# niclasborlin/dbat

Hardware: AMD Instinct MI355X
Metric: LM iterations/sec (higher is better)
Workload: dtype f64

## Files before the change

### dbat_amd/csrc/dbat_core.hip

```cpp
#include <hip/hip_runtime.h>
#include <rocblas/rocblas.h>
#include <rocsolver/rocsolver.h>
#include <rccl/rccl.h>

#include <chrono>
#include <cmath>
#include <cstdio>
#include <cstdlib>
#include <memory>
#include <string>
#include <thread>
#include <type_traits>
#include <utility>
#include <atomic>
#include <vector>

#include "../../include/dbat_hip.h"
#include "chol_df.hpp"
#include "kernels.hpp"
#include "sig.hpp"
#include "heavy.hpp"
#include "plan.hpp"
#include "resect.hpp"
#include "robust.hpp"
// ... 156 lines not shown
        if (lds > 65536) {
            int i = 0;
            while (i < n_lds_opt_in && lds_opt_in[i].kernel != (const void *)K) ++i;
            if (i == n_lds_opt_in || lds_opt_in[i].bytes < lds) {
                if (i == 8) throw DeviceError{"internal: more kernels with over 64 KiB of LDS than the opt-in table holds"};
                HIPCHK(hipFuncSetAttribute((const void *)K, hipFuncAttributeMaxDynamicSharedMemorySize, (int)lds));
                lds_opt_in[i] = {(const void *)K, lds};
                n_lds_opt_in = std::max(n_lds_opt_in, i + 1);
            }
        }
        dbat::launch<K>(grid, block, lds, stream, std::forward<A>(args)...);
    }
    double f_lin = 0, trace_jtj = 0, lambda_lin = 0;
    int scale_lin = 0;
    bool have_lin = false;
    bool s_valid = false;
    bool s_dense_dirty = true;
    int n_res_evals = 0, n_lin = 0, n_solves = 0, n_trace_only = 0;

    ~Core() {
        for (auto &e : ev) if (e) (void)hipEventDestroy(e);
        for (auto &e : kev) if (e) (void)hipEventDestroy(e);
        for (auto &e : st_ev) if (e) (void)hipEventDestroy(e);
        dfchol.release(); dfchol_ip.release();
        if (hpin) (void)hipHostFree(hpin);
        if (nccl) (void)ncclCommDestroy(nccl);
        if (blas) rocblas_destroy_handle(blas);
        if (stream) (void)hipStreamDestroy(stream);
    }

// ... 73 lines not shown
            hv.io_dst = hv_io_dst.p; hv.io_ld = hv_io_ld.p; hv.io_pt = hv_io_pt.p; hv.pt_y = hv_pt_y.p;
            hv.grp_nb = hv_grp_nb.p; hv.grp_row = hv_grp_row.p; hv.task = hv_task.p; hv.ops = hv_ops.p;
            hv.obs0 = P.hv_obs0; hv.pt0 = P.hv_pt0; hv.ntasks = P.hv_ntasks; hv.max_batch_slots = P.hv_max_batch_slots;
        }
        if (const char *e = env_get("DBAT_HIP_GIANT_THREADS")) giant_threads = atoi(e);
        d.tile_batch = tile_batch.p; d.tile_cam_start = tile_cam_start.p; d.tile_cams = tile_cams.p;
        d.tile_io_start = tile_io_start.p; d.tile_iocols = tile_iocols.p; d.tile_cam_io = tile_cam_io.p;
        tile_io_simple.upload(P.tile_io_simple); d.tile_io_simple = P.tile_io_simple.empty() ? nullptr : tile_io_simple.p;
        use_sig = P.sg_ok && ntiles > 0 && tile_ncx <= 14;
        if (use_sig) {
            sg_chunk.upload(P.sg_chunk); sg_tile_chunk0.upload(P.sg_tile_chunk0); sg_lc.upload(P.sg_lc); sg_gcam.upload(P.sg_gcam);
            sg_nchunks = (int64_t)P.sg_chunk.size() / 8;
            sg_uv.upload(P.sg_uv);
            if (!P.uniform_w) sg_w.upload(P.sg_w);
            sig_rb = P.sg_rows_max <= 64 ? 4 : 5;
        }
        lapi("allocations and uploads of the plan");
        cams.alloc(P.nc); cams_f.alloc(P.nc);
        z.alloc(P.NZ); zt.alloc(P.NZ); dz.alloc(P.NZ); zlin.alloc(P.NZ); vtmp.alloc(P.NZ); vtmp2.alloc(P.NZ);
        xbuf.alloc(std::max<int64_t>(P.n, 1));
        ldS = ((P.NS + 1 + 7) / 8) * 8;
        d.ldS = ldS;
        const int64_t s_count = ldS * (P.NS + 1);
        red_count = s_count + 3 * P.NS + 8;
        red.alloc(red_count);
        S = red.p; g_red = S + s_count; g_c = g_red + P.NS; diagU = g_c + P.NS; red_scal = diagU + P.NS;
        ldiag.alloc(P.NS);
        {
            std::vector<int> first((size_t)P.NS, 0);
            for (int c = 0; c < P.nc; ++c)
                for (int k = 0; k < 6; ++k) first[(size_t)6 * c + k] = 6 * P.cam_first[c];
// ... 84 lines not shown
        robust_reset();
        HIPCHK(hipMemcpyAsync(z.p, P.z0.data(), P.NZ * 8, hipMemcpyHostToDevice, stream));
        HIPCHK(hipMemcpyAsync(io_fixed.p, P.io_fixed.data(), P.io_fixed.size() * 8, hipMemcpyHostToDevice, stream));
        if (d.any_prior) {
            HIPCHK(hipMemcpyAsync(z_prw.p, P.z_prw.data(), P.NZ * 8, hipMemcpyHostToDevice, stream));
            HIPCHK(hipMemcpyAsync(z_prv.p, P.z_prv.data(), P.NZ * 8, hipMemcpyHostToDevice, stream));
        }
        HIPCHK(hipStreamSynchronize(stream));
        if (uv_pre && io_changed && nobs > 0) {
            HIPCHK(hipMemcpy(cm_uv.p, P.cm_uv.data(), P.cm_uv.size() * 8, hipMemcpyHostToDevice));
            if (use_sig && sg_nchunks > 0) HIPCHK(hipMemcpy(sg_uv.p, P.sg_uv.data(), P.sg_uv.size() * 8, hipMemcpyHostToDevice));
            d.o_uv = o_uv.p;
            precompute_image_side();
            HIPCHK(hipStreamSynchronize(stream));
        }
        cams_at_lin = false; have_lin = false; s_valid = false; pend_build = false; lin_pending = false;
        lambda_lin = 0; scale_lin = 0; f_lin = 0; trace_jtj = 0; near_singular = false; chol_in_place = false; replicate_next = false;
        n_res_evals = n_lin = n_solves = n_trace_only = 0;
    }

    static int env_grid_obs() { return std::min(std::max(1, env_int("DBAT_HIP_GRID_OBS", 1536)), 1 << 20); }

    int64_t tile_kernel_mfma() const {
        if (route == TileRoute::none) return 0;
        int64_t n = 0;
        if (route == TileRoute::sig) {
            for (int64_t t = 0; t < ntiles; ++t) {
                const int nio = tile_ncx > 6 ? P.tile_io_start[t + 1] - P.tile_io_start[t] : 0;
                for (int64_t q = P.sg_tile_chunk0[t]; q < P.sg_tile_chunk0[t + 1]; ++q) {
                    const int npts = P.sg_chunk[8 * q + 1], k = P.sg_chunk[8 * q + 2];
                    const int ppr = std::min(SIG_PPR, 64 / std::max(k, 1)), rbk = (6 * k + nio + 1 + 15) >> 4;
// ... 95 lines not shown
    void read_scal(double *host, int n) {
        if (n <= 32) {
            HIPCHK(hipMemcpyAsync(hpin, scal.p, n * sizeof(double), hipMemcpyDeviceToHost, stream));
            sync();
            memcpy(host, hpin, n * sizeof(double));
            return;
        }
        HIPCHK(hipMemcpyAsync(host, scal.p, n * sizeof(double), hipMemcpyDeviceToHost, stream));
        sync();
    }
    void prep_cams(const double *zz, CamRec *into = nullptr) {
        if (!into) { into = cams.p; cams_at_lin = false; }
        launch<k_cam_prep>(dim3((unsigned)cdiv(P.nc, 64)), dim3(64), 0, d, zz, into);
    }
    void x_to_z(const double *x_host, double *z_dev) {
        HIPCHK(hipMemcpyAsync(z_dev, P.z0.data(), P.NZ * 8, hipMemcpyHostToDevice, stream));
        if (P.n) {
            HIPCHK(hipMemcpyAsync(xbuf.p, x_host, P.n * 8, hipMemcpyHostToDevice, stream));
            launch<k_scatter_x>(dim3((unsigned)cdiv(P.n, 256)), dim3(256), 0, P.n, x2z.p, xbuf.p, z_dev);
        }
    }
    void z_to_x(const double *z_dev, double *x_host) {
        if (!P.n) return;
        stage(4);
        z_dev = gathered(z_dev);
        launch<k_gather_x>(dim3((unsigned)cdiv(P.n, 256)), dim3(256), 0, P.n, x2z.p, z_dev, xbuf.p);
        HIPCHK(hipMemcpyAsync(x_host, xbuf.p, P.n * 8, hipMemcpyDeviceToHost, stream));
        sync();
    }

// ... 25 lines not shown
        if (!P.n || nt <= 0) return std::max(nt, 0);
        HIPCHK(hipMemcpyAsync(host, trace_dev.p, (size_t)P.n * nt * 8, hipMemcpyDeviceToHost, stream));
        HIPCHK(hipStreamSynchronize(stream));
        for (int k = 0; k < nt; ++k)
            if (!trace_have[k]) std::fill(host + (size_t)P.n * k, host + (size_t)P.n * (k + 1), NAN);
        if ((size_t)P.n * trace_cap * 8 > ((size_t)256 << 20)) {
            DevBuf<double> old;
            std::swap(old.p, trace_dev.p);
            trace_cap = 0;
        }
        return nt;
    }

    double eval_f_step(const double *x, double alpha, const double *pdir, double *out) {
        stage(3);
        if ((int64_t)cdiv(P.NZ, 256) < P.nc) { axpby(1.0, x, alpha, pdir, out); return eval_f(out, nullptr, nullptr); }
        launch<k_axpby_cams>(dim3((unsigned)cdiv(P.NZ, 256)), dim3(256), 0, d, 1.0, x, alpha, pdir, out, cams_f.p);
        return eval_f(out, nullptr, nullptr, true);
    }
    double eval_f(const double *zz, double *r_w_out, double *r_unw_out, bool cams_ready = false) {
        stage(3);
        if (!cams_ready) prep_cams(zz, cams_f.p);
        mark(6);
        const bool res_tail = n_cm_chunks_all > 0 && n_cm_chunks_all <= 512 && !d.any_prior && !multi() && !r_w_out && !r_unw_out;
        with_value<2, 3, 4, 5>(P.model, [&](auto M) {
            with_value<false, true>(uv_pre, [&](auto PRE) {
                if (n_cm_chunks_all > 0)
                    launch<k_residual_cm<M, PRE>>(dim3((unsigned)n_cm_chunks_all), dim3(256), 0, d, zz, cams_f.p, cm_pt.p, cm_uv.p, pw ? cm_w.p : (const double *)nullptr,
                                                  cm_chunk_cam.p, cm_chunk_start.p, partial.p, res_tail ? gctr.p + 1 : (unsigned *)nullptr, scal.p, hpin, res_tail ? ++mb_seq : 0ull);
                mark(7);
// ... 52 lines not shown
        else launch<k_det_round_cam<15>>(dim3((unsigned)P.nc + 1), dim3(256), 0, d, cams.p, nio, S, g_red);
    }

    void cam_normal(const double *zz, int64_t q0, int64_t nq, int ncx) {
        const double *w = pw ? cm_w.p : (const double *)nullptr;
        with_value<2, 3, 4, 5>(P.model, [&](auto M) { with_value<6, 14, 15>(ncx, [&](auto NCX) {
            if constexpr (NCX == 6)
                launch<k_cam_normal6<M>>(dim3((unsigned)nq), dim3(256), 0, d, zz, cams.p, cm_pt.p, cm_uv.p, w, cm_chunk_cam.p + q0, cm_chunk_start.p + q0, S, g_c, g_red, diagU);
            else
                launch<k_cam_normal<M, NCX>>(dim3((unsigned)nq), dim3(256), 0, d, zz, cams.p, cm_pt.p, cm_uv.p, w, cm_chunk_cam.p + q0, cm_chunk_start.p + q0, S, g_c, g_red, diagU);
        }); });
    }

    void build_enqueue(const double *zz, double lambda, int scale) {
        stage(0);
        const bool fused_first = !s_dense_dirty && P.NS >= P.nc;
        if (!fused_first) prep_cams(zz);
        else cams_at_lin = false;
        bool pivmm_set = false;
        if (s_dense_dirty) {
            HIPCHK(hipMemsetAsync(red.p, 0, red_count * sizeof(double), stream));
            s_dense_dirty = false;
        } else {
            launch<k_envelope_cams>(dim3((unsigned)P.NS), dim3(256), 0, d, zz, cams.p, S, ldS, (int)P.NS, env_tail0, col_bend.p, g_red, pivmm.p);
            pivmm_set = true;
        }
        if (!pivmm_set) HIPCHK(hipMemcpyAsync(pivmm.p, hpin + 48, 4 * sizeof(double), hipMemcpyHostToDevice, stream));
        int64_t npart = 0;
        const bool det_list = deterministic && route != TileRoute::sig;
        const int64_t nb_tiled = det_list ? 0 : P.nb_tiled;
// ... 124 lines not shown
        do_allreduce(g_c, 2 * P.NS + 8);
    }
    void trace_only_pass(const double *zz) {
        stage(0);
        prep_cams(zz);
        if (n_cm_chunks_all > 0) {
            with_value<2, 3, 4, 5>(P.model, [&](auto M) { with_value<6, 14, 15, MAXCOL>(tile_ncx, [&](auto NCX) {
                launch<k_trace_cm<M, NCX>>(dim3((unsigned)n_cm_chunks_all), dim3(256), 0, d, zz, cams.p, cm_pt.p, cm_uv.p, pw ? cm_w.p : (const double *)nullptr,
                                           cm_chunk_cam.p, cm_chunk_start.p, partial.p);
            }); });
        }
        launch<k_trace_tail>(dim3(grid_zs), dim3(1024), 0, d, gpart.p, gctr.p + 6, (const double *)partial.p, n_cm_chunks_all, hpin, ++mb_seq);
        mb_armed = true; lin_pending = true;
        sync();
        pend_build = false;
        lambda_lin = NAN; have_lin = false; s_valid = false;
        ++n_trace_only;
    }
    void build(const double *zz, double lambda, int scale, bool lazy = false, bool trace_only = false) {
        if (trace_only && !multi() && P.nranks == 1) { trace_only_pass(zz); return; }
        pend_build = false;
        trace_only = trace_only && use_sig && ntiles > 0;
        d.trace_only = trace_only ? 1 : 0;
        try { build_enqueue(zz, lambda, scale); } catch (...) { d.trace_only = 0; throw; }
        d.trace_only = 0;
        if (mg_subtree) allreduce_vectors();
        else allreduce_system();
        finish_enqueue(zz, lambda, scale);
        if (mg_subtree && replicate_next && multi()) allreduce_matrix();
        cams_at_lin = true;
        lin_pending = true;
// ... 17 lines not shown
        launch<k_finish>(dim3((unsigned)cdiv(P.NS, 256)), dim3(256), 0, d, zz, lambda, scale, S, g_c, g_red, diagU, jn2c.p, dscale.p,
                gpart.p, gctr.p + 3, (const double *)red_scal, scal.p, hpin, mg_subtree && multi() ? (const uint8_t *)z_mine.p : (const uint8_t *)nullptr,
                ride ? info.p : (int *)nullptr, ride ? df_ctl : (int *)nullptr, ride ? df_q : (unsigned long long *)nullptr, ride ? df_nq : 0);
        if (ride) dfchol.reset_done = true;
        if (scale)
            launch<k_envelope_op>(dim3((unsigned)P.NS), dim3(256), 0, S, ldS, (int)P.NS, env_tail0, col_bend.p, (const double *)dscale.p, (double *)nullptr,
                                  (unsigned long long *)nullptr);
    }

    int factor_solve_enqueue() {
        if (mg_subtree && !multi())
            throw UsageError{"this handle is one of several shards: attach a communicator (dbat_hip_comm_init) or an all-reduce "
                             "callback (dbat_hip_set_allreduce) before linearising or solving"};
        stage(1);
        mark(2);
        if (use_perm && !chol_in_place && mg_subtree && multi()) {
            dfchol.solve_domain(stream, S, ldS, linv.p, info.p, ldiag.p);
            mark(8);
            do_allreduce(dfchol.top_tiles(), dfchol.top_tiles_count());
            mark(9);
            dfchol.solve_top(stream, ldS, rhs.p, linv.p, info.p, ldiag.p, dscale.p, dz.p);
        } else if (use_perm && !chol_in_place) dfchol.solve(stream, S, ldS, rhs.p, linv.p, info.p, ldiag.p, dscale.p, dz.p);
        else dfchol_ip.solve(stream, S, ldS, rhs.p, linv.p, info.p, ldiag.p, dscale.p, dz.p);
        HIPCHK(hipGetLastError());
        if (env_df_trace) (use_perm && !chol_in_place ? dfchol : dfchol_ip).dump_trace(stream, env_df_trace);
        mark(3);
        ++n_solves;
        return 0;
    }
    void backsub_enqueue() {
        stage(2);
        mark(4);
        const bool sig_bs = use_sig && P.sg_backsub_ok;
        const int64_t b_first = sig_bs ? P.nb_tiled : 0;
        const int64_t n_sig_wg = sig_bs ? cdiv(sg_nchunks, 4) : 0;
        if (n_sig_wg > 0) {
            with_value<2, 3, 4, 5>(P.model, [&](auto M) { with_value<6, 14>(tile_ncx, [&](auto NCX) {
                launch<k_backsub_sig<M, NCX>>(dim3((unsigned)n_sig_wg), dim3(256), 0, d, zlin.p, cams.p, Vinv.p, gp.p, dz.p, partial.p + 2 * (nb + ngiant), sg_chunk.p,
                                              (int)sg_nchunks, sg_gcam.p, sg_uv.p, pw ? sg_w.p : (const double *)nullptr);
            }); });
        }
        if (nb > b_first) {
            with_value<2, 3, 4, 5>(P.model, [&](auto M) { with_value<6, 14, 15, MAXCOL>(tile_ncx, [&](auto NCX) {
                launch<k_backsub<M, NCX>>(dim3((unsigned)(nb - b_first)), dim3(P.BT), lds_back, d, zlin.p, cams.p, Vinv.p, gp.p, dz.p, partial.p, (int)b_first);
            }); });
        }
        if (ngiant > 0) {
            with_value<2, 3, 4, 5>(P.model, [&](auto M) { with_value<false, true>(P.with_io, [&](auto IO) {
                launch<k_backsub_giant<M, IO>>(dim3((unsigned)ngiant), dim3(giant_threads), 0, d, zlin.p, cams.p, Vinv.p, gp.p, dz.p, partial.p + 2 * nb);
            }); });
        }
        mark(5);
        launch<k_prior_jv>(dim3(grid_zs), dim3(1024), 0, d, zlin.p, dz.p, g_c, gp.p, gpart.p, gctr.p + 4,
                (const double *)(partial.p + 2 * b_first), nb - b_first + ngiant + n_sig_wg, (const double *)ldiag.p, pivmm.p,
                (const int *)info.p, scal.p, multi() ? (double *)nullptr : hpin, ++mb_seq,
                mg_subtree && multi() ? (const uint8_t *)piv_have.p : (const uint8_t *)nullptr);
    }
    bool near_singular = false;
    const bool pivot_stats = env_on("DBAT_HIP_PIVOT_STATS");
    double rcond_est = 0.0;
    int chol_info = 0;
    double piv_last[4] = {0, 0, 0, 0};
    bool solve(double &JpJp, double &rJp, double &pp) {
        ensure_build();
        if (!s_valid) build(zlin.p, lambda_lin, scale_lin);
        s_valid = false;
        factor_solve_enqueue();
        if (!cams_at_lin) { prep_cams(zlin.p); cams_at_lin = true; }
        backsub_enqueue();
        int hinfo = 0;
        unsigned long long hmm[4];
        const int nsl = multi() ? 4 * P.nranks : 0;
        std::vector<double> h((size_t)8 + nsl);
        if (nsl) {
            HIPCHK(hipMemcpyAsync(hpin + 40, pivmm.p, sizeof(hmm), hipMemcpyDeviceToHost, stream));
            HIPCHK(hipMemcpyAsync(hpin + 44, info.p, sizeof(hinfo), hipMemcpyDeviceToHost, stream));
            HIPCHK(hipMemsetAsync(scal.p + 8, 0, (size_t)nsl * sizeof(double), stream));
            HIPCHK(hipMemcpyAsync(scal.p + 8 + 4 * P.rank, pivmm.p, 4 * sizeof(double), hipMemcpyDeviceToDevice, stream));
            do_allreduce(scal.p, 8 + nsl);
            read_scal(h.data(), 8 + nsl);
        } else {
            mb_armed = true;
            sync();
            memcpy(h.data(), hpin, 8 * sizeof(double));
        }
        memcpy(hmm, hpin + 40, sizeof(hmm));
        memcpy(&hinfo, hpin + 44, sizeof(hinfo));
        JpJp = h[0] + h[4]; rJp = h[1] + h[5]; pp = h[6];
        double mm[4];
        memcpy(mm, hmm, sizeof(mm));
        double pmin = std::min(mm[0], mm[2]), pmax = std::max(mm[1], mm[3]);
        for (int r = 0; r < nsl / 2; ++r) { pmin = std::min(pmin, h[8 + 2 * r]); pmax = std::max(pmax, h[8 + 2 * r + 1]); }
        const bool failed = hinfo != 0 || (nsl && h[7] > 0) || !std::isfinite(pp) || !std::isfinite(JpJp);
        if (failed && !(use_perm && !chol_in_place)) s_dense_dirty = true;
        const double ratio = pmax > 0 ? pmin / pmax : 0.0;
        near_singular = failed || !(ratio * ratio >= 2.220446049250313e-16);
        rcond_est = failed ? 0.0 : ratio * ratio;
        chol_info = hinfo;
        for (int q = 0; q < 4; ++q) piv_last[q] = mm[q];
// ... 363 lines not shown
    void robust_omega_ip(double *host) {
        if (!robust_on) { std::fill(host, host + P.no, 1.0); return; }
        DevBuf<double> t;
        t.alloc((size_t)std::max<int64_t>(P.no, 1));
        HIPCHK(hipMemsetAsync(t.p, 0, (size_t)P.no * sizeof(double), stream));
        if (nobs > 0) launch<k_scatter_rows1>(dim3(robust_grid()), dim3(256), 0, nobs, (const int64_t *)o_row.p, (const double *)omega.p, t.p);
        if (multi()) do_allreduce(t.p, P.no);
        HIPCHK(hipMemcpyAsync(host, t.p, (size_t)P.no * sizeof(double), hipMemcpyDeviceToHost, stream));
        HIPCHK(hipStreamSynchronize(stream));
    }
    void jtimes(const double *v, double &JvJv, double &rJv, double &vv) {
        if (!cams_at_lin) { prep_cams(zlin.p); cams_at_lin = true; }
        with_value<2, 3, 4, 5>(P.model, [&](auto M) { with_value<6, 14, 15, MAXCOL>(tile_ncx, [&](auto NCX) {
            launch<k_jtimes<M, NCX>>(dim3(grid_obs), dim3(256), 0, d, zlin.p, cams.p, v, partial.p);
        }); });
        launch<k_prior_jv>(dim3(grid_zs), dim3(1024), 0, d, zlin.p, v, g_c, gp.p, gpart.p, gctr.p + 4,
                (const double *)partial.p, (int64_t)grid_obs, (const double *)nullptr, pivmm.p, (const int *)info.p, scal.p, (double *)nullptr, 0ull, (const uint8_t *)nullptr);
        do_allreduce(scal.p, 8);
        double h[8];
        read_scal(h, 8);
        JvJv = h[0] + h[4]; rJv = h[1] + h[5]; vv = h[6];
    }
    double dot_owned(const double *a, const double *b) {
        launch<k_dot>(dim3(grid_z), dim3(256), 0, P.NZ, z_mine.p, a, b, partial.p);
        launch<k_sum_partials<1>>(dim3(1), dim3(1024), 0, partial.p, (int64_t)grid_z, scal.p, 0);
        do_allreduce(scal.p, 1);
        double s;
        read_scal(&s, 1);
        return s;
    }
    void axpby(double a, const double *x, double b, const double *y2, double *y) {
        launch<k_axpby>(dim3((unsigned)cdiv(P.NZ, 256)), dim3(256), 0, P.NZ, a, x, b, y2, y);
    }
    void gradient(double *g) {
        launch<k_gradient>(dim3((unsigned)cdiv(P.NZ, 256)), dim3(256), 0, d, g_c, gp.p, g);
    }
    void colnorm2(double *out) {
        launch<k_jn2>(dim3((unsigned)cdiv(P.NZ, 256)), dim3(256), 0, d, jn2c.p, jn2p.p, out);
    }
    void jac_blocks(const double *zz, double *a, double *b, double *cc) {
        with_value<2, 3, 4, 5>(P.model, [&](auto M) { launch<k_jac_blocks<M>>(dim3((unsigned)cdiv(nobs, 256)), dim3(256), 0, d, zz, cams.p, a, b, cc); });
    }
    void copy(double *dst, const double *src) { HIPCHK(hipMemcpyAsync(dst, src, P.NZ * 8, hipMemcpyDeviceToDevice, stream)); }
    void accept_trial() { std::swap(z.p, zt.p); }
};


struct LoopOut {
    std::vector<double> res, damp, aux;
    int code = 0, iters = 0;
    double f_final = 0;
};

static void export_residuals(Core &c, const double *zdev, double *r_unw, double *r_wgt, double *f);
static void jtimes_rows(Core &c, const double *v_dev, double *Jv);

static void keep_Jp(Core &c, const dbat_hip_options &o, const double *p_dev, std::vector<double> &Jp) {
    if (!o.term_fun) return;
    Jp.resize((size_t)c.P.m);
// ... 95 lines not shown
    double f = c.eval_f(c.z.p, nullptr, nullptr);
    c.build(c.z.p, 0.0, 0, false, lambda0_needs_trace(o));
    const double nx = (double)c.P.n;
    double lambda0 = o.lambda0, lambdaMin = o.lambda_min;
    if (lambda0 < 0) lambda0 = std::fabs(lambda0) * c.trace_jtj / nx;
    if (lambdaMin < 0) lambdaMin = std::fabs(lambdaMin) * c.trace_jtj / nx;
    double lambda = lambda0;
    if (lambda < lambdaMin) lambda = 0;
    out.damp.push_back(lambda);
    double prevLambda = NAN;
    double JpJp = 0, rJp = 0, pp = 0;
    std::vector<double> Jp_host;
    while (true) {
        while (n <= o.max_iter) {
            if (c.lambda_lin != lambda) c.build(c.z.p, lambda, 0, true);
            const bool failed = c.solve(JpJp, rJp, pp);
            if (!failed) keep_Jp(c, o, c.dz.p, Jp_host);
            out.res.push_back(std::sqrt(2 * f));
            if (n == 0 && !c.P.rank_ok) { out.code = -4; break; }
            if (failed) { out.code = -2; break; }
            out.damp.push_back(lambda);
            trace_line(o, n, out.res.back(), n == 0 ? NAN : lambda);
            if (o.store_trace) c.trace_put(n, c.z.p);
            ++n;
            const double fNew = c.eval_f_step(c.z.p, 1.0, c.dz.p, c.zt.p);
            if (fNew < f && !vetoed(c, o)) {
                c.accept_trial();
                lambda = lambda / 10;
                if (lambda < lambdaMin) lambda = 0;
                c.request_build(lambda, 0);
                f = fNew;
// ... 17 lines not shown
static void loop_lmp(Core &c, const dbat_hip_options &o, double delta0, LoopOut &out) {
    int n = 0;
    double delta = delta0;
    std::vector<double> rhos, steps;
    if (o.store_trace) c.trace_put(0, c.z.p);
    double f = c.eval_f(c.z.p, nullptr, nullptr);
    c.build(c.z.p, 0.0, 1);
    bool have_gn = false;
    std::vector<double> Jp_host;
    double gnJpJp = 0, gnrJp = 0, gnpp = 0;
    double *pGN = c.vtmp.p, *g = c.vtmp2.p;
    while (true) {
        out.res.push_back(std::sqrt(2 * f));
        if (n == 0 && !c.P.rank_ok) { out.code = -4; break; }
        if (!have_gn) {
            const bool failed = c.solve(gnJpJp, gnrJp, gnpp);
            if (failed) { out.code = -2; break; }
            c.copy(pGN, c.dz.p);
            have_gn = true;
        }
        int step;
        double JpJp, rJp;
        const double npGN = std::sqrt(gnpp);
        if (npGN <= delta) {
            step = 0; c.copy(c.dz.p, pGN); JpJp = gnJpJp; rJp = gnrJp;
        } else {
            c.gradient(g);
            double gJJg, rJg, gg;
            c.jtimes(g, gJJg, rJg, gg);
            const double lambdaStar = gg / gJJg;
            const double nCP = lambdaStar * std::sqrt(gg);
            if (nCP > delta) {
                step = 2;
                c.axpby(-delta / std::sqrt(gg), g, 0.0, g, c.dz.p);
            } else {
                step = 1;
                const double cp_pgn = -lambdaStar * c.dot_owned(g, pGN);
                const double cp2 = nCP * nCP;
                const double A = cp2 - 2 * cp_pgn + gnpp;
                const double B = 2 * (cp_pgn - cp2);
// ... 831 lines not shown
}

int dbat_hip_bench_step(dbat_hip_handle *h, double lambda, int32_t scale_columns, double *ms) {
    API_TRY
    if (!h) { g_err = "null handle"; return DBAT_HIP_EINVAL; }
    Core &c = *h->core;
    DeviceGuard dev_guard(c.device);
    c.timing = true;
    HIPCHK(hipEventRecord(c.ev[0], c.stream));
    c.build_enqueue(c.z.p, lambda, scale_columns);
    if (c.mg_subtree) c.allreduce_vectors(); else c.allreduce_system();
    c.finish_enqueue(c.z.p, lambda, scale_columns);
    HIPCHK(hipEventRecord(c.ev[1], c.stream));
    c.factor_solve_enqueue();
    HIPCHK(hipEventRecord(c.ev[2], c.stream));
    c.backsub_enqueue();
    c.do_allreduce(c.scal.p, 8);
    HIPCHK(hipEventRecord(c.ev[3], c.stream));
    (void)c.eval_f_step(c.z.p, 1.0, c.dz.p, c.zt.p);
    HIPCHK(hipEventRecord(c.ev[4], c.stream));
    c.sync();
    c.timing = false;
    c.have_lin = true; c.lambda_lin = lambda; c.scale_lin = scale_columns; c.s_valid = false;
    if (ms) {
        for (int i = 0; i < 4; ++i) {
            float t = 0;
            HIPCHK(hipEventElapsedTime(&t, c.ev[i], c.ev[i + 1]));
            ms[i] = t;
        }
        for (int i = 0; i < 4; ++i) {
            float t = 0;
// ... 391 lines not shown
```

### dbat_amd/csrc/env.hpp

```cpp
#pragma once
#include <cstdlib>
#include <cstring>
#include <string>

extern char **environ;

namespace dbat {

#ifdef DBAT_HIP_PROFILING
constexpr bool kProfilingBuild = true;
#else
constexpr bool kProfilingBuild = false;
#endif

struct EnvSwitch { const char *name; bool measurement; const char *what; const char *values = nullptr; };
static const EnvSwitch kEnvSwitches[] = {
    {"DBAT_HIP_SIG", false, "0: signature kernels off, 2: on wherever a chunk's rows fit (default: by group length)", "0|1|2"},
    {"DBAT_HIP_SIG_IOS_OFF", false, "self-calibration: IO rows by LDS atomics in every tile"},
    {"DBAT_HIP_CMAX", false, "cameras per tile (0: column-list kernel only)"},
    {"DBAT_HIP_BT", false, "observations per batch (128 | 256)", "128|256"},
    {"DBAT_HIP_TILE_BMIN", false, "fewest batches a tile may be capped at (default 2)"},
    {"DBAT_HIP_HEAVY", false, "0: heavy / giant points by the column-list kernels (pair terms by global atomics) instead of the matrix-core path", "0|1"},
    {"DBAT_HIP_HEAVY_KS", false, "heavy / giant points: k-steps per task of k_heavy_syrk at most (default: by the amount of work, 12 ... 96)"},
    {"DBAT_HIP_GIANT_THREADS", false, "threads of the giant-point kernels (64 | 128 | 256)", "64|128|256"},
    {"DBAT_HIP_MG_REPLICATED", false, "several ranks: envelope summed, replicated factorisation"},
    {"DBAT_HIP_ND_OFF", false, "no nested dissection"},
    {"DBAT_HIP_ND_LEAF", false, "leaf size of the dissection"},
    {"DBAT_HIP_ND_PAD_ALL", false, "every block of the dissection on a tile boundary"},
    {"DBAT_HIP_ND_JOIN_SMALL", false, "separators up to that many rows join their child's last tile"},
    {"DBAT_HIP_DF_SPLIT", false, "factorisation: helper tasks for sums longer than this many products (default 96)"},
    {"DBAT_HIP_DF_CHUNK", false, "factorisation: products per helper task (default 32)"},
    {"DBAT_HIP_DF_CHAIN", false, "factorisation: 0 = diagonal tiles as ordinary tasks (no chain role), 1 = chain role whatever the pattern", "0|1"},
// ... 50 lines not shown
```

### dbat_amd/csrc/kernels.hpp

```cpp
#pragma once
#include <hip/hip_runtime.h>

#include "model.hpp"

namespace dbat {

struct DevProblem {
    int nc, np, nIOrows, nK, nP, nIOu, ncolmax, BT;
    int64_t NS, NZ, nobs, nb;
    int64_t ldS;
    const int32_t *cam_ncol, *cam_col, *cam_iorow;
    const uint32_t *cam_eo_est;
    const int32_t *io_src;
    const double *io_fixed;
    const double *px;
    const double *cam_w;
    const uint8_t *z_est, *z_mine;
    const double *z_prw, *z_prv;
    const int32_t *o_cam, *o_pt;
    const double *o_uv;
    const double *o_uv_raw;
    int uv_pre;
    const double *o_w;
    const uint32_t *o_seg;
// ... 2678 lines not shown
    const int cam = d.o_cam[o], pt = d.o_pt[o];
    const CamRec &C = cams[cam];
    const int ncol = WITH_IO ? min(C.ncol, NCX) : 6;
    double r[2], E[2][NCX], B[2][3];
    eval_obs_cols_n<MODEL, NCX>(d, C, z, o, pt, r, E, B);
    const double *vp = v + d.NS + 3 * (int64_t)pt;
    double j0 = B[0][0] * vp[0] + B[0][1] * vp[1] + B[0][2] * vp[2];
    double j1 = B[1][0] * vp[0] + B[1][1] * vp[1] + B[1][2] * vp[2];
#pragma unroll
    for (int a = 0; a < NCX; ++a)
        if (a < ncol) { const double vc = v[C.col[a]]; j0 += E[0][a] * vc; j1 += E[1][a] * vc; }
    const int64_t row = d.o_row[o];
    Jv[2 * row] = j0; Jv[2 * row + 1] = j1;
}

__global__ __launch_bounds__(1024) void k_prior_jv(DevProblem d, const double *__restrict__ z,
                                                  const double *__restrict__ v, const double *__restrict__ g_c,
                                                  const double *__restrict__ gp, double *__restrict__ partial,
                                                  unsigned *__restrict__ ctr, const double *__restrict__ bs_partial,
                                                  int64_t nbs, const double *__restrict__ ldiag,
                                                  unsigned long long *__restrict__ pivmm, const int *__restrict__ info,
                                                  double *__restrict__ out, double *__restrict__ mailbox,
                                                  unsigned long long seq, const uint8_t *__restrict__ piv_have = nullptr) {
    __shared__ double sh[80];
    double acc[5] = {0, 0, 0, 0, 0};
    const int64_t stride = (int64_t)gridDim.x * blockDim.x;
    double pmin = 1e300, pmax = 0.0;
    for (int64_t i = (int64_t)blockIdx.x * blockDim.x + threadIdx.x; i < d.NZ; i += stride) {
        if (ldiag && i < d.NS && d.z_est[i] && (!piv_have || piv_have[i])) {
            double p = ldiag[i];
            p = p == p ? p : 0.0;
            pmin = fmin(pmin, p); pmax = fmax(pmax, p);
        }
        if (!d.z_mine[i]) continue;
        const double w = d.any_prior ? d.z_prw[i] : 0.0, vi = d.z_est[i] ? v[i] : 0.0;
        if (w > 0) acc[0] += w * vi * vi;
        acc[1] += (i < d.NS ? g_c[i] : gp[i - d.NS]) * vi;
        acc[2] += vi * vi;
    }
    if (ldiag && (int64_t)blockIdx.x * blockDim.x < d.NS) {
        for (int off = 32; off > 0; off >>= 1) {
            pmin = fmin(pmin, __shfl_down(pmin, off, 64));
            pmax = fmax(pmax, __shfl_down(pmax, off, 64));
        }
        if ((threadIdx.x & 63) == 0 && pmax > 0.0) {
            atomicMin(pivmm + 2, (unsigned long long)__double_as_longlong(fmax(pmin, 0.0)));
            atomicMax(pivmm + 3, (unsigned long long)__double_as_longlong(pmax));
        }
        __builtin_amdgcn_s_waitcnt(0);
    }
    if (grid_sum<5, 2, 3>(acc, sh, partial, ctr, bs_partial, nbs, 2) && threadIdx.x == 0) {
        out[0] = acc[3]; out[1] = acc[4]; out[4] = acc[0]; out[5] = acc[1]; out[6] = acc[2];
        out[7] = info && __hip_atomic_load(info, __ATOMIC_RELAXED, __HIP_MEMORY_SCOPE_AGENT) != 0 ? 1.0 : 0.0;
        out[2] = 0.0; out[3] = 0.0;
        if (mailbox) {
            mailbox[0] = acc[3]; mailbox[1] = acc[4]; mailbox[4] = acc[0]; mailbox[5] = acc[1]; mailbox[6] = acc[2];
            for (int q = 0; q < 4; ++q)
                mailbox[40 + q] = __longlong_as_double((long long)__hip_atomic_load(pivmm + q, __ATOMIC_RELAXED, __HIP_MEMORY_SCOPE_AGENT));
            const int hi = __hip_atomic_load(info, __ATOMIC_RELAXED, __HIP_MEMORY_SCOPE_AGENT);
            long long w = hi;
            mailbox[44] = __longlong_as_double(w);
            mailbox_done(mailbox, seq);
        }
    }
}

__global__ __launch_bounds__(256) void k_dot(int64_t n, const uint8_t *__restrict__ mine,
                                             const double *__restrict__ a, const double *__restrict__ b ,
                                             double *__restrict__ partial) {
    __shared__ double sh[8];
// ... 4 lines not shown
    block_sum<1>(acc, sh);
    if (threadIdx.x == 0) partial[blockIdx.x] = acc[0];
}

__global__ void k_axpby(int64_t n, double a, const double *__restrict__ x, double b,
                        const double *__restrict__ y2, double *__restrict__ y) {
    const int64_t i = (int64_t)blockIdx.x * blockDim.x + threadIdx.x;
    if (i < n) y[i] = a * x[i] + b * y2[i];
}
__global__ void k_axpby_cams(DevProblem d, double a, const double *__restrict__ x, double b,
                             const double *__restrict__ y2, double *__restrict__ y, CamRec *__restrict__ cams) {
    const int64_t i = (int64_t)blockIdx.x * blockDim.x + threadIdx.x;
    if (i < d.NZ) y[i] = a * x[i] + b * y2[i];
    if (threadIdx.x == blockDim.x - 1 && (int)blockIdx.x < d.nc)
        cam_prep_one(d, [=](int64_t q) { return a * x[q] + b * y2[q]; }, (int)blockIdx.x, cams);
}

__global__ void k_gradient(DevProblem d, const double *__restrict__ g_c, const double *__restrict__ gp,
                           double *__restrict__ g) {
    const int64_t i = (int64_t)blockIdx.x * blockDim.x + threadIdx.x;
    if (i >= d.NZ) return;
    double v = 0;
    if (d.z_est[i]) v = i < d.NS ? g_c[i] : (d.z_mine[i] ? gp[i - d.NS] : 0.0);
    g[i] = v;
}

__global__ void k_jn2(DevProblem d, const double *__restrict__ jn2c, const double *__restrict__ jn2p,
                      double *__restrict__ out) {
    const int64_t i = (int64_t)blockIdx.x * blockDim.x + threadIdx.x;
    if (i >= d.NZ) return;
// ... 64 lines not shown
```

### dbat_amd/csrc/sig.hpp

```cpp
#pragma once
#include <cstddef>
#include <type_traits>

#include "kernels.hpp"

namespace dbat {

constexpr int SIG_LDK = 18;
constexpr int SIG_PPR = 6;
constexpr int SIG_KMAXR = 13;
constexpr int SIG_NW = 8;
constexpr int SIG_CAMW = (int)(offsetof(CamRec, ncol) / 8) + 1;
constexpr int SIG_CAMW_IO = (int)((sizeof(CamRec) + 7) / 8);
constexpr int SIG_STILE = 8064;
#ifndef DBAT_SIG_IO_WAVES
#define DBAT_SIG_IO_WAVES 4
#endif
constexpr int SIG_IO_CAMS = DBAT_SIG_IO_WAVES == 8 ? 16 : 21;
__host__ __device__ constexpr int sig_stile(bool io) { return io && DBAT_SIG_IO_WAVES == 8 ? 6336 : SIG_STILE; }
__host__ __device__ constexpr int sig_cams(bool io) { return io ? SIG_IO_CAMS : 21; }

struct SigLds {
    int next_chunk, abort_;
    int flush_turn;
// ... 655 lines not shown
        int ios = 0;
        if constexpr (NCX > 6) ios = d.tile_io_simple ? d.tile_io_simple[tile] : 0;
#ifdef DBAT_SIG_ONLY_IOS
        ios = DBAT_SIG_ONLY_IOS;
#endif
        if (NCX > 6 && ios == 1)
            build_sig_tile<MODEL, RB, NCX, (NCX > 6 ? 1 : 0), PW>(d, tile, (int)ti, z, cams, lambda, scale, S, g_red, Vinv, gp, jn2p, partial, pivmm, sg_chunk, sg_tile_chunk0, sg_lc, sg_uv, sg_w, tile_ctr + 2, sy, sh);
        else if (NCX > 6 && ios == 2)
            build_sig_tile<MODEL, RB, NCX, (NCX > 6 ? 2 : 0), PW>(d, tile, (int)ti, z, cams, lambda, scale, S, g_red, Vinv, gp, jn2p, partial, pivmm, sg_chunk, sg_tile_chunk0, sg_lc, sg_uv, sg_w, tile_ctr + 2, sy, sh);
        else
            build_sig_tile<MODEL, RB, NCX, 0, PW>(d, tile, (int)ti, z, cams, lambda, scale, S, g_red, Vinv, gp, jn2p, partial, pivmm, sg_chunk, sg_tile_chunk0, sg_lc, sg_uv, sg_w, tile_ctr + 2, sy, sh);
        __syncthreads();
    }
}

template <int MODEL, int NCX>
__global__ __launch_bounds__(256) void k_backsub_sig(DevProblem d, const double *__restrict__ z,
                                                     const CamRec *__restrict__ cams,
                                                     const double *__restrict__ Vinv, const double *__restrict__ gp,
                                                     double *__restrict__ dz, double *__restrict__ partial ,
                                                     const int32_t *__restrict__ sg_chunk, int nchunks,
                                                     const int32_t *__restrict__ sg_gcam,
                                                     const double *__restrict__ sg_uv, const double *__restrict__ sg_w) {
    constexpr int CW = (int)((sizeof(CamRec) + 7) / 8);
    __shared__ double sh[8];
    __shared__ double crec[4][SIG_KMAXR][CW];
    __shared__ double dcs[4][SIG_KMAXR][NCX];
    const int t = threadIdx.x, lane = t & 63;
    const int wv = t >> 6;
    const int ch = __builtin_amdgcn_readfirstlane(blockIdx.x * 4 + (t >> 6));
    double acc[2] = {0, 0};
    if (ch < nchunks) {
        const int32_t *cd = sg_chunk + 8 * (int64_t)ch;
        const int pt0 = cd[0], npts = cd[1], k = cd[2], gm = cd[4], gi0 = cd[5], uv0 = cd[6];
        const int mycam = lane < k ? sg_gcam[16 * (int64_t)ch + lane] : 0;
        for (int base = 0; base < k * CW; base += 64) {
            const int idx = base + lane, c = min(idx / CW, k - 1), f = idx - c * CW;
            const int cam = __builtin_amdgcn_ds_bpermute(4 * c, mycam);
            if (idx < k * CW) crec[wv][c][f] = reinterpret_cast<const double *>(cams + cam)[f];
        }
        __builtin_amdgcn_wave_barrier();
        for (int idx = lane; idx < k * NCX; idx += 64) {
            const int c = idx / NCX, a = idx - c * NCX;
            const CamRec &C = *reinterpret_cast<const CamRec *>(crec[wv][c]);
            const bool on = a < (NCX > 6 ? min(C.ncol, NCX) : 6) && (NCX > 6 || ((C.eo_est >> a) & 1u));
            dcs[wv][c][a] = on ? dz[C.col[a]] : 0.0;
// ... 44 lines not shown
#pragma unroll
            for (int c = 0; c < 6; ++c) V0[c] += lane_get(V0[c], lane ^ m);
            tt2 += lane_get(tt2, lane ^ m);
        }
        {
            const double s0 = gp[3 * (int64_t)pt] + sB[0], s1 = gp[3 * (int64_t)pt + 1] + sB[1], s2 = gp[3 * (int64_t)pt + 2] + sB[2];
            double p0, p1, p2;
            point_block_solve_neg(Vinv + 6 * (int64_t)pt, s0, s1, s2, p0, p1, p2);
            const double d0 = (est & 1u) ? p0 : 0.0, d1 = (est & 2u) ? p1 : 0.0, d2 = (est & 4u) ? p2 : 0.0;
            if (act && lane == pi) {
                dz[zp] = d0; dz[zp + 1] = d1; dz[zp + 2] = d2;
                acc[0] = tt2 + 2.0 * (d0 * sB[0] + d1 * sB[1] + d2 * sB[2])
                       + d0 * (V0[0] * d0 + V0[1] * d1 + V0[2] * d2) + d1 * (V0[1] * d0 + V0[3] * d1 + V0[4] * d2)
                       + d2 * (V0[2] * d0 + V0[4] * d1 + V0[5] * d2);
            }
        }
    }
    block_sum<2>(acc, sh);
    if (t == 0) { partial[2 * blockIdx.x] = acc[0]; partial[2 * blockIdx.x + 1] = acc[1]; }
}

}
```

Measured before the change: 634.4.

## Fuse trial-step objective evaluation into signature back-substitution kernel

When the solve is followed by a full-step objective evaluation, the back-substitution kernel now also forms the trial point coordinates, re-evaluates the residuals at the trial cameras and points, and accumulates the trial objective, with the prior term added in the prior/Jv reduction kernel. A small kernel prepares trial camera records before the back-substitution. The later eval_f_step call then reads the cached value from the mailbox instead of launching separate residual kernels, saving a pass over the observations and a host round trip. Validity flags are reset on every path that modifies z, dz, zt or the linearisation, which adds state-tracking complexity and puts extra work and register pressure on the back-substitution kernel.

```diff
diff --git a/dbat_amd/csrc/dbat_core.hip b/dbat_amd/csrc/dbat_core.hip
--- a/dbat_amd/csrc/dbat_core.hip
+++ b/dbat_amd/csrc/dbat_core.hip
@@ -194,6 +194,10 @@
     double f_lin = 0, trace_jtj = 0, lambda_lin = 0;
     int scale_lin = 0;
     bool have_lin = false;
+    bool trial_ok = false, trial_read = false;
+    double trial_f = 0;
+    bool fused_trial = true;
+    bool sg_all_points = false;
     bool s_valid = false;
     bool s_dense_dirty = true;
     int n_res_evals = 0, n_lin = 0, n_solves = 0, n_trace_only = 0;
@@ -297,7 +301,11 @@
             sg_uv.upload(P.sg_uv);
             if (!P.uniform_w) sg_w.upload(P.sg_w);
             sig_rb = P.sg_rows_max <= 64 ? 4 : 5;
-        }
+            int64_t npts = 0;
+            for (int64_t q = 0; q < sg_nchunks; ++q) npts += P.sg_chunk[8 * q + 1];
+            sg_all_points = npts == (int64_t)P.np;
+        }
+        fused_trial = env_int("DBAT_HIP_FUSED_TRIAL", 1) != 0;
         lapi("allocations and uploads of the plan");
         cams.alloc(P.nc); cams_f.alloc(P.nc);
         z.alloc(P.NZ); zt.alloc(P.NZ); dz.alloc(P.NZ); zlin.alloc(P.NZ); vtmp.alloc(P.NZ); vtmp2.alloc(P.NZ);
@@ -412,7 +420,7 @@
             precompute_image_side();
             HIPCHK(hipStreamSynchronize(stream));
         }
-        cams_at_lin = false; have_lin = false; s_valid = false; pend_build = false; lin_pending = false;
+        cams_at_lin = false; have_lin = false; trial_ok = false; s_valid = false; pend_build = false; lin_pending = false;
         lambda_lin = 0; scale_lin = 0; f_lin = 0; trace_jtj = 0; near_singular = false; chol_in_place = false; replicate_next = false;
         n_res_evals = n_lin = n_solves = n_trace_only = 0;
     }
@@ -538,6 +546,7 @@
         launch<k_cam_prep>(dim3((unsigned)cdiv(P.nc, 64)), dim3(64), 0, d, zz, into);
     }
     void x_to_z(const double *x_host, double *z_dev) {
+        trial_ok = false;
         HIPCHK(hipMemcpyAsync(z_dev, P.z0.data(), P.NZ * 8, hipMemcpyHostToDevice, stream));
         if (P.n) {
             HIPCHK(hipMemcpyAsync(xbuf.p, x_host, P.n * 8, hipMemcpyHostToDevice, stream));
@@ -593,6 +602,13 @@
 
     double eval_f_step(const double *x, double alpha, const double *pdir, double *out) {
         stage(3);
+        if (trial_ok && alpha == 1.0 && x == z.p && pdir == dz.p && out == zt.p) {
+            mark(6); mark(7);
+            if (!trial_read) { mb_armed = true; sync(); trial_f = hpin[8]; trial_read = true; }
+            ++n_res_evals;
+            return 0.5 * trial_f;
+        }
+        trial_ok = false;
         if ((int64_t)cdiv(P.NZ, 256) < P.nc) { axpby(1.0, x, alpha, pdir, out); return eval_f(out, nullptr, nullptr); }
         launch<k_axpby_cams>(dim3((unsigned)cdiv(P.NZ, 256)), dim3(256), 0, d, 1.0, x, alpha, pdir, out, cams_f.p);
         return eval_f(out, nullptr, nullptr, true);
@@ -675,6 +691,7 @@
 
     void build_enqueue(const double *zz, double lambda, int scale) {
         stage(0);
+        trial_ok = false;
         const bool fused_first = !s_dense_dirty && P.NS >= P.nc;
         if (!fused_first) prep_cams(zz);
         else cams_at_lin = false;
@@ -829,7 +846,7 @@
         mb_armed = true; lin_pending = true;
         sync();
         pend_build = false;
-        lambda_lin = NAN; have_lin = false; s_valid = false;
+        lambda_lin = NAN; have_lin = false; trial_ok = false; s_valid = false;
         ++n_trace_only;
     }
     void build(const double *zz, double lambda, int scale, bool lazy = false, bool trace_only = false) {
@@ -877,6 +894,7 @@
                              "callback (dbat_hip_set_allreduce) before linearising or solving"};
         stage(1);
         mark(2);
+        trial_ok = false;
         if (use_perm && !chol_in_place && mg_subtree && multi()) {
             dfchol.solve_domain(stream, S, ldS, linv.p, info.p, ldiag.p);
             mark(8);
@@ -891,16 +909,26 @@
         ++n_solves;
         return 0;
     }
-    void backsub_enqueue() {
+    bool trial_fusable() const {
+        return fused_trial && use_sig && P.sg_backsub_ok && sg_nchunks > 0 && sg_all_points && nb == P.nb_tiled && ngiant == 0 &&
+               (tile_ncx == 6) == uv_pre && !deterministic && !multi() && P.nranks == 1;
+    }
+    void backsub_enqueue(bool want_trial = false) {
         stage(2);
         mark(4);
+        const bool fuse = want_trial && trial_fusable();
+        trial_ok = false;
+        if (fuse) launch<k_trial_cams>(dim3((unsigned)cdiv(P.NS, 256)), dim3(256), 0, d, zlin.p, dz.p, zt.p, cams_f.p);
         const bool sig_bs = use_sig && P.sg_backsub_ok;
         const int64_t b_first = sig_bs ? P.nb_tiled : 0;
         const int64_t n_sig_wg = sig_bs ? cdiv(sg_nchunks, 4) : 0;
         if (n_sig_wg > 0) {
             with_value<2, 3, 4, 5>(P.model, [&](auto M) { with_value<6, 14>(tile_ncx, [&](auto NCX) {
-                launch<k_backsub_sig<M, NCX>>(dim3((unsigned)n_sig_wg), dim3(256), 0, d, zlin.p, cams.p, Vinv.p, gp.p, dz.p, partial.p + 2 * (nb + ngiant), sg_chunk.p,
-                                              (int)sg_nchunks, sg_gcam.p, sg_uv.p, pw ? sg_w.p : (const double *)nullptr);
+                with_value<false, true>(fuse, [&](auto TR) {
+                    launch<k_backsub_sig<M, NCX, TR>>(dim3((unsigned)n_sig_wg), dim3(256), 0, d, zlin.p, cams.p, Vinv.p, gp.p, dz.p, partial.p + 2 * (nb + ngiant), sg_chunk.p,
+                                                      (int)sg_nchunks, sg_gcam.p, sg_uv.p, pw ? sg_w.p : (const double *)nullptr,
+                                                      TR ? zt.p : (double *)nullptr, TR ? cams_f.p : (const CamRec *)nullptr);
+                });
             }); });
         }
         if (nb > b_first) {
@@ -914,23 +942,26 @@
             }); });
         }
         mark(5);
-        launch<k_prior_jv>(dim3(grid_zs), dim3(1024), 0, d, zlin.p, dz.p, g_c, gp.p, gpart.p, gctr.p + 4,
-                (const double *)(partial.p + 2 * b_first), nb - b_first + ngiant + n_sig_wg, (const double *)ldiag.p, pivmm.p,
-                (const int *)info.p, scal.p, multi() ? (double *)nullptr : hpin, ++mb_seq,
-                mg_subtree && multi() ? (const uint8_t *)piv_have.p : (const uint8_t *)nullptr);
+        with_value<false, true>(fuse, [&](auto TR) {
+            launch<k_prior_jv<TR>>(dim3(grid_zs), dim3(1024), 0, d, zlin.p, dz.p, g_c, gp.p, gpart.p, gctr.p + 4,
+                    (const double *)(partial.p + 2 * b_first), nb - b_first + ngiant + n_sig_wg, (const double *)ldiag.p, pivmm.p,
+                    (const int *)info.p, scal.p, multi() ? (double *)nullptr : hpin, ++mb_seq,
+                    mg_subtree && multi() ? (const uint8_t *)piv_have.p : (const uint8_t *)nullptr);
+        });
+        trial_ok = fuse; trial_read = false;
     }
     bool near_singular = false;
     const bool pivot_stats = env_on("DBAT_HIP_PIVOT_STATS");
     double rcond_est = 0.0;
     int chol_info = 0;
     double piv_last[4] = {0, 0, 0, 0};
-    bool solve(double &JpJp, double &rJp, double &pp) {
+    bool solve(double &JpJp, double &rJp, double &pp, bool want_trial = false) {
         ensure_build();
         if (!s_valid) build(zlin.p, lambda_lin, scale_lin);
         s_valid = false;
         factor_solve_enqueue();
         if (!cams_at_lin) { prep_cams(zlin.p); cams_at_lin = true; }
-        backsub_enqueue();
+        backsub_enqueue(want_trial);
         int hinfo = 0;
         unsigned long long hmm[4];
         const int nsl = multi() ? 4 * P.nranks : 0;
@@ -946,6 +977,7 @@
             mb_armed = true;
             sync();
             memcpy(h.data(), hpin, 8 * sizeof(double));
+            if (trial_ok) { trial_f = hpin[8]; trial_read = true; }
         }
         memcpy(hmm, hpin + 40, sizeof(hmm));
         memcpy(&hinfo, hpin + 44, sizeof(hinfo));
@@ -1339,7 +1371,7 @@
         with_value<2, 3, 4, 5>(P.model, [&](auto M) { with_value<6, 14, 15, MAXCOL>(tile_ncx, [&](auto NCX) {
             launch<k_jtimes<M, NCX>>(dim3(grid_obs), dim3(256), 0, d, zlin.p, cams.p, v, partial.p);
         }); });
-        launch<k_prior_jv>(dim3(grid_zs), dim3(1024), 0, d, zlin.p, v, g_c, gp.p, gpart.p, gctr.p + 4,
+        launch<k_prior_jv<false>>(dim3(grid_zs), dim3(1024), 0, d, zlin.p, v, g_c, gp.p, gpart.p, gctr.p + 4,
                 (const double *)partial.p, (int64_t)grid_obs, (const double *)nullptr, pivmm.p, (const int *)info.p, scal.p, (double *)nullptr, 0ull, (const uint8_t *)nullptr);
         do_allreduce(scal.p, 8);
         double h[8];
@@ -1355,6 +1387,7 @@
         return s;
     }
     void axpby(double a, const double *x, double b, const double *y2, double *y) {
+        trial_ok = false;
         launch<k_axpby>(dim3((unsigned)cdiv(P.NZ, 256)), dim3(256), 0, P.NZ, a, x, b, y2, y);
     }
     void gradient(double *g) {
@@ -1366,8 +1399,11 @@
     void jac_blocks(const double *zz, double *a, double *b, double *cc) {
         with_value<2, 3, 4, 5>(P.model, [&](auto M) { launch<k_jac_blocks<M>>(dim3((unsigned)cdiv(nobs, 256)), dim3(256), 0, d, zz, cams.p, a, b, cc); });
     }
-    void copy(double *dst, const double *src) { HIPCHK(hipMemcpyAsync(dst, src, P.NZ * 8, hipMemcpyDeviceToDevice, stream)); }
-    void accept_trial() { std::swap(z.p, zt.p); }
+    void copy(double *dst, const double *src) {
+        if (dst == z.p || dst == zt.p || dst == dz.p || dst == zlin.p) trial_ok = false;
+        HIPCHK(hipMemcpyAsync(dst, src, P.NZ * 8, hipMemcpyDeviceToDevice, stream));
+    }
+    void accept_trial() { std::swap(z.p, zt.p); trial_ok = false; }
 };
 
 
@@ -1493,7 +1529,7 @@
     while (true) {
         while (n <= o.max_iter) {
             if (c.lambda_lin != lambda) c.build(c.z.p, lambda, 0, true);
-            const bool failed = c.solve(JpJp, rJp, pp);
+            const bool failed = c.solve(JpJp, rJp, pp, true);
             if (!failed) keep_Jp(c, o, c.dz.p, Jp_host);
             out.res.push_back(std::sqrt(2 * f));
             if (n == 0 && !c.P.rank_ok) { out.code = -4; break; }
@@ -1541,7 +1577,7 @@
         out.res.push_back(std::sqrt(2 * f));
         if (n == 0 && !c.P.rank_ok) { out.code = -4; break; }
         if (!have_gn) {
-            const bool failed = c.solve(gnJpJp, gnrJp, gnpp);
+            const bool failed = c.solve(gnJpJp, gnrJp, gnpp, true);
             if (failed) { out.code = -2; break; }
             c.copy(pGN, c.dz.p);
             have_gn = true;
@@ -1550,7 +1586,8 @@
         double JpJp, rJp;
         const double npGN = std::sqrt(gnpp);
         if (npGN <= delta) {
-            step = 0; c.copy(c.dz.p, pGN); JpJp = gnJpJp; rJp = gnrJp;
+            step = 0; JpJp = gnJpJp; rJp = gnrJp;
+            if (!c.trial_ok) c.copy(c.dz.p, pGN);
         } else {
             c.gradient(g);
             double gJJg, rJg, gg;
@@ -2412,7 +2449,7 @@
     HIPCHK(hipEventRecord(c.ev[1], c.stream));
     c.factor_solve_enqueue();
     HIPCHK(hipEventRecord(c.ev[2], c.stream));
-    c.backsub_enqueue();
+    c.backsub_enqueue(true);
     c.do_allreduce(c.scal.p, 8);
     HIPCHK(hipEventRecord(c.ev[3], c.stream));
     (void)c.eval_f_step(c.z.p, 1.0, c.dz.p, c.zt.p);
diff --git a/dbat_amd/csrc/env.hpp b/dbat_amd/csrc/env.hpp
--- a/dbat_amd/csrc/env.hpp
+++ b/dbat_amd/csrc/env.hpp
@@ -16,6 +16,7 @@
 struct EnvSwitch { const char *name; bool measurement; const char *what; const char *values = nullptr; };
 static const EnvSwitch kEnvSwitches[] = {
     {"DBAT_HIP_SIG", false, "0: signature kernels off, 2: on wherever a chunk's rows fit (default: by group length)", "0|1|2"},
+    {"DBAT_HIP_FUSED_TRIAL", false, "0: the objective at the full step by its own kernels behind the solve, not inside the back-substitution", "0|1"},
     {"DBAT_HIP_SIG_IOS_OFF", false, "self-calibration: IO rows by LDS atomics in every tile"},
     {"DBAT_HIP_CMAX", false, "cameras per tile (0: column-list kernel only)"},
     {"DBAT_HIP_BT", false, "observations per batch (128 | 256)", "128|256"},
diff --git a/dbat_amd/csrc/kernels.hpp b/dbat_amd/csrc/kernels.hpp
--- a/dbat_amd/csrc/kernels.hpp
+++ b/dbat_amd/csrc/kernels.hpp
@@ -2716,6 +2716,7 @@
     Jv[2 * row] = j0; Jv[2 * row + 1] = j1;
 }
 
+template <bool TRIAL>
 __global__ __launch_bounds__(1024) void k_prior_jv(DevProblem d, const double *__restrict__ z,
                                                   const double *__restrict__ v, const double *__restrict__ g_c,
                                                   const double *__restrict__ gp, double *__restrict__ partial,
@@ -2724,8 +2725,9 @@
                                                   unsigned long long *__restrict__ pivmm, const int *__restrict__ info,
                                                   double *__restrict__ out, double *__restrict__ mailbox,
                                                   unsigned long long seq, const uint8_t *__restrict__ piv_have = nullptr) {
-    __shared__ double sh[80];
-    double acc[5] = {0, 0, 0, 0, 0};
+    constexpr int NV = TRIAL ? 6 : 5;
+    __shared__ double sh[16 * NV];
+    double acc[NV] = {};
     const int64_t stride = (int64_t)gridDim.x * blockDim.x;
     double pmin = 1e300, pmax = 0.0;
     for (int64_t i = (int64_t)blockIdx.x * blockDim.x + threadIdx.x; i < d.NZ; i += stride) {
@@ -2739,6 +2741,8 @@
         if (w > 0) acc[0] += w * vi * vi;
         acc[1] += (i < d.NS ? g_c[i] : gp[i - d.NS]) * vi;
         acc[2] += vi * vi;
+        if constexpr (TRIAL)
+            if (w > 0) { const double e = (z[i] + v[i]) - d.z_prv[i]; acc[5] += w * e * e; }
     }
     if (ldiag && (int64_t)blockIdx.x * blockDim.x < d.NS) {
         for (int off = 32; off > 0; off >>= 1) {
@@ -2751,11 +2755,12 @@
         }
         __builtin_amdgcn_s_waitcnt(0);
     }
-    if (grid_sum<5, 2, 3>(acc, sh, partial, ctr, bs_partial, nbs, 2) && threadIdx.x == 0) {
+    if (grid_sum<NV, NV - 3, 3>(acc, sh, partial, ctr, bs_partial, nbs, NV - 3) && threadIdx.x == 0) {
         out[0] = acc[3]; out[1] = acc[4]; out[4] = acc[0]; out[5] = acc[1]; out[6] = acc[2];
         out[7] = info && __hip_atomic_load(info, __ATOMIC_RELAXED, __HIP_MEMORY_SCOPE_AGENT) != 0 ? 1.0 : 0.0;
-        out[2] = 0.0; out[3] = 0.0;
+        out[2] = TRIAL ? acc[NV - 1] : 0.0; out[3] = 0.0;
         if (mailbox) {
+            if constexpr (TRIAL) mailbox[8] = acc[NV - 1];
             mailbox[0] = acc[3]; mailbox[1] = acc[4]; mailbox[4] = acc[0]; mailbox[5] = acc[1]; mailbox[6] = acc[2];
             for (int q = 0; q < 4; ++q)
                 mailbox[40 + q] = __longlong_as_double((long long)__hip_atomic_load(pivmm + q, __ATOMIC_RELAXED, __HIP_MEMORY_SCOPE_AGENT));
@@ -2790,6 +2795,14 @@
     if (i < d.NZ) y[i] = a * x[i] + b * y2[i];
     if (threadIdx.x == blockDim.x - 1 && (int)blockIdx.x < d.nc)
         cam_prep_one(d, [=](int64_t q) { return a * x[q] + b * y2[q]; }, (int)blockIdx.x, cams);
+}
+
+__global__ __launch_bounds__(256) void k_trial_cams(DevProblem d, const double *__restrict__ x,
+                                                    const double *__restrict__ p, double *__restrict__ y,
+                                                    CamRec *__restrict__ cams) {
+    const int64_t i = (int64_t)blockIdx.x * blockDim.x + threadIdx.x;
+    if (i < d.NS) y[i] = x[i] + p[i];
+    if (i < d.nc) cam_prep_one(d, [=](int64_t q) { return x[q] + p[q]; }, (int)i, cams);
 }
 
 __global__ void k_gradient(DevProblem d, const double *__restrict__ g_c, const double *__restrict__ gp,
diff --git a/dbat_amd/csrc/sig.hpp b/dbat_amd/csrc/sig.hpp
--- a/dbat_amd/csrc/sig.hpp
+++ b/dbat_amd/csrc/sig.hpp
@@ -693,22 +693,24 @@
     }
 }
 
-template <int MODEL, int NCX>
+template <int MODEL, int NCX, bool TRIAL = false>
 __global__ __launch_bounds__(256) void k_backsub_sig(DevProblem d, const double *__restrict__ z,
                                                      const CamRec *__restrict__ cams,
                                                      const double *__restrict__ Vinv, const double *__restrict__ gp,
                                                      double *__restrict__ dz, double *__restrict__ partial ,
                                                      const int32_t *__restrict__ sg_chunk, int nchunks,
                                                      const int32_t *__restrict__ sg_gcam,
-                                                     const double *__restrict__ sg_uv, const double *__restrict__ sg_w) {
+                                                     const double *__restrict__ sg_uv, const double *__restrict__ sg_w,
+                                                     double *__restrict__ zt = nullptr, const CamRec *__restrict__ cams_t = nullptr) {
     constexpr int CW = (int)((sizeof(CamRec) + 7) / 8);
-    __shared__ double sh[8];
+    constexpr int NP = TRIAL ? 3 : 2;
+    __shared__ double sh[4 * NP];
     __shared__ double crec[4][SIG_KMAXR][CW];
     __shared__ double dcs[4][SIG_KMAXR][NCX];
     const int t = threadIdx.x, lane = t & 63;
     const int wv = t >> 6;
     const int ch = __builtin_amdgcn_readfirstlane(blockIdx.x * 4 + (t >> 6));
-    double acc[2] = {0, 0};
+    double acc[NP] = {};
     if (ch < nchunks) {
         const int32_t *cd = sg_chunk + 8 * (int64_t)ch;
         const int pt0 = cd[0], npts = cd[1], k = cd[2], gm = cd[4], gi0 = cd[5], uv0 = cd[6];
@@ -783,10 +785,41 @@
                        + d0 * (V0[0] * d0 + V0[1] * d1 + V0[2] * d2) + d1 * (V0[1] * d0 + V0[3] * d1 + V0[4] * d2)
                        + d2 * (V0[2] * d0 + V0[4] * d1 + V0[5] * d2);
             }
-        }
-    }
-    block_sum<2>(acc, sh);
-    if (t == 0) { partial[2 * blockIdx.x] = acc[0]; partial[2 * blockIdx.x + 1] = acc[1]; }
+            if constexpr (TRIAL) {
+                const double Qt[3] = {Q[0] + d0, Q[1] + d1, Q[2] + d2};
+                if (act && lane == pi) { zt[zp] = Qt[0]; zt[zp + 1] = Qt[1]; zt[zp + 2] = Qt[2]; }
+                __builtin_amdgcn_wave_barrier();
+                for (int base = 0; base < k * CW; base += 64) {
+                    const int idx = base + lane, c = min(idx / CW, k - 1), f = idx - c * CW;
+                    const int cam = __builtin_amdgcn_ds_bpermute(4 * c, mycam);
+                    if (idx < k * CW) crec[wv][c][f] = reinterpret_cast<const double *>(cams_t + cam)[f];
+                }
+                __builtin_amdgcn_wave_barrier();
+                double rr = 0;
+                auto sweep_t = [&](auto per_obs_w) {
+                for (int j = jh; j < k; j += jstep) {
+                    const CamRec &C = *reinterpret_cast<const CamRec *>(crec[wv][j]);
+                    const double2 uv = uvp[q0 + (int64_t)j * gm];
+                    double w0, w1;
+                    if constexpr (decltype(per_obs_w)::value) { const double2 ww = wp[q0 + (int64_t)j * gm]; w0 = ww.x; w1 = ww.y; }
+                    else { w0 = C.w[0]; w1 = C.w[1]; }
+                    double r[2];
+                    double(*nil6)[6] = nullptr; double(*nil3)[3] = nullptr; double(*nilc)[MAXIO] = nullptr;
+                    obs_eval<MODEL, false, false, (NCX == 6)>(C, d.nK, d.nP, Qt, uv.x, uv.y, r, nil6, nil3, nilc);
+                    r[0] *= w0; r[1] *= w1;
+                    rr += r[0] * r[0] + r[1] * r[1];
+                }
+                };
+                if (sg_w) sweep_t(std::true_type{}); else sweep_t(std::false_type{});
+                if (act) acc[NP - 1] = rr;
+            }
+        }
+    }
+    block_sum<NP>(acc, sh);
+    if (t == 0) {
+#pragma unroll
+        for (int i = 0; i < NP; ++i) partial[NP * blockIdx.x + i] = acc[i];
+    }
 }
 
 }
```

Result: slower. 621.9 (-2.0%).
